# sparisi/pvr_habitat

Hardware: AMD Instinct MI355X
Metric: frames/sec embedded (ResNet50, 256x256) (higher is better)
Workload: dtype f16; 1 GPU; configs[1]: ResNet50 (MoCo-v2 layout) frozen, 256x256 uint8 frames resident in HBM, batch 256/GPU, random-init synthetic weights, f16 storage / MFMA inputs with fp32 accumulation (the product default, inside the 1e-3 parity bound; configs[1] names bf16); global_batch=256, frame=256, chunk=256, batches_in_flight=2, parallelism=frame shards, no collective (dp1)

## Files before the change

pvr_habitat_amd/csrc/bottleneck_chain.hip:

```cpp
#include "encoder_internal.h"

namespace pvr {


__device__ __forceinline__ void ch_dma16(__amdgpu_buffer_rsrc_t rs, char *lds, int voff, int soff) {
    __builtin_amdgcn_raw_ptr_buffer_load_lds(rs, (__attribute__((address_space(3))) void *)lds, 16, voff, soff, 0, 0);
}

#ifdef CHAIN_STAMP
__device__ unsigned long long chain_stamps[8192][12];
#define CH_T(i_) { if (threadIdx.x == 0) ch_tt[i_] = __builtin_amdgcn_s_memrealtime(); }
#else
#define CH_T(i_)
#endif

#ifndef CH_KNOCK
#define CH_KNOCK 0
#endif
template <int AUX = 0>
__device__ __forceinline__ void store_b128_imm(u32x4 v, __amdgpu_buffer_rsrc_t rs, int voff, int imm) {
    if constexpr (!(CH_KNOCK & 1)) __builtin_amdgcn_raw_buffer_store_b128(v, rs, voff + imm, 0, AUX);
}

template <int CM, int CMN, bool F16, int RD, int OCC, bool HALO, bool DS = false, int PFK = -1>
__global__ __launch_bounds__(256, OCC) void bottleneck_chain_kernel(ChainP p) {
    typedef typename HT<F16>::V8 V8;
    constexpr int BM = 128, BK = 64, BN = CM;
    constexpr int A_CH = BM / 32, B_CH = BN / 32, TM = 4, TN = BN / 32;
    constexpr int KS = CM / 64, HROWS = CM == 64 ? 256 : 192, RL = CM == 64 ? 3 : 2;
    constexpr int HSL = HROWS * 128, RING_OFF = KS * HSL, SLICE = CM * 128, ZERO_OFF = (HROWS - 1) * 128;
    constexpr int HOPS = KS * HROWS / 32;
    constexpr int STAGE = HALO ? (RING_OFF + 2 * SLICE) / 2 : (BM + BN) * 128;
    constexpr int C4 = 4 * CM, G = C4 / 64, KS3 = CM / 64;
    constexpr int TN1 = CMN / 32;
    constexpr int W3_CH = CM / 32, W1_CH = CMN / 32;
    constexpr int T2_OFF = 0;
    constexpr int YG_OFF = KS3 * 16384;
    constexpr int W3_OFF = YG_OFF + 16384;
    constexpr int W1_OFF = W3_OFF + KS3 * 8192;
    static_assert(W3_OFF + KS3 * 8192 <= 2 * STAGE, "phase-B tiles must fit the phase-A area");
    static_assert(RD >= 1 && RD <= G, "residual prefetch depth");
    extern __shared__ __attribute__((aligned(16))) char smem[];

    const int tid = threadIdx.x, lane = tid & 63, wave = tid >> 6;
#ifdef CHAIN_STAMP
    unsigned long long ch_tt[12] = {0, 0, 0, 0, 0, 0, 0, 0, 0, 0, 0, 0};
#endif
    CH_T(0);
    const int m0 = xcd_remap(blockIdx.x, gridDim.x) * BM;
    const int srow = tid >> 3, pch = tid & 7;
    const auto rs_in = __builtin_amdgcn_make_buffer_rsrc(const_cast<u16 *>(p.in), 0, p.in_bytes, 0x00020000);
    const auto rs_w2 = __builtin_amdgcn_make_buffer_rsrc(const_cast<u16 *>(p.w2), 0, p.w2_bytes, 0x00020000);
    const auto rs_w3 = __builtin_amdgcn_make_buffer_rsrc(const_cast<u16 *>(p.w3), 0, p.w3_bytes, 0x00020000);
    const auto rs_w1 = __builtin_amdgcn_make_buffer_rsrc(const_cast<u16 *>(p.w1n), 0, p.w1n_bytes, 0x00020000);
    const auto rs_res = __builtin_amdgcn_make_buffer_rsrc(const_cast<u16 *>(DS ? p.xds : p.res), 0, DS ? p.xds_bytes : p.y_bytes, 0x00020000);
    const auto rs_wd = __builtin_amdgcn_make_buffer_rsrc(const_cast<u16 *>(DS ? p.wds : p.w3), 0, DS ? p.wds_bytes : p.w3_bytes, 0x00020000);
    const auto rs_y = __builtin_amdgcn_make_buffer_rsrc(p.y, 0, p.y_bytes, 0x00020000);
    const auto rs_t = __builtin_amdgcn_make_buffer_rsrc(p.t1n, 0, p.t1n_bytes, 0x00020000);
    constexpr int OOB = 0x7ffffff0;

    if constexpr (HALO) {
        const int HR = 128 + 2 * p.W + 2, hbase = m0 - p.W - 1;
#pragma unroll
        for (int i = 0; i < HOPS; ++i) {
            const int o = i * 4 + wave, sl = o / (HROWS / 8), rb = o % (HROWS / 8);
            const int r = rb * 8 + (lane >> 3), c = (lane & 7) ^ (r & 6);
            const int vo = (r < HR && hbase + r >= 0) ? ((hbase + r) * CM + sl * 64 + c * 8) * 2 : OOB;
            ch_dma16(rs_in, smem + sl * HSL + rb * 1024, vo, 0);
        }
    }

    int a_off[A_CH], a_mask[A_CH];
#pragma unroll
    for (int i = 0; i < A_CH; ++i) {
        const int row = srow + 32 * i;
        const int lch = pch ^ ((row >> 1) & 7);
        const int m = m0 + row;
        const bool ok = m < p.M;
        const int mm = ok ? m : 0;
        const int wo = mm % p.Wo, t = mm / p.Wo, ho = t % p.Ho, n = t / p.Ho;
        const int hi0 = ho * p.stride - 1, wi0 = wo * p.stride - 1;
        a_off[i] = (((n * p.H + hi0) * p.W + wi0) * CM + lch * 8) * 2;
        int hb = 0, wb = 0;
#pragma unroll
        for (int t3 = 0; t3 < 3; ++t3) {
            hb |= (int)(ok && (unsigned)(hi0 + t3) < (unsigned)p.H) << t3;
            wb |= (int)((unsigned)(wi0 + t3) < (unsigned)p.W) << t3;
        }
        int mask = 0;
#pragma unroll
        for (int t3 = 0; t3 < 3; ++t3) mask |= ((hb >> t3) & 1) ? (wb << (t3 * 3)) : 0;
        a_mask[i] = mask;
    }
    int b_off[B_CH];
#pragma unroll
    for (int i = 0; i < B_CH; ++i) {
        const int row = srow + 32 * i;
        b_off[i] = (row * (9 * CM) + (pch ^ ((row >> 1) & 7)) * 8) * 2;
    }
    const int lds_st = srow * 128 + pch * 16;
    u32x4 ra[A_CH], rb[B_CH];
    constexpr int cpt = CM / BK, nk = 9 * cpt;
    int kh = 0, kw = 0, cs = 0, tap = 0;
#define PVR_LOAD_SLICE(kt_)                                                                             \
    {                                                                                                   \
        const int tap_off = ((kh * p.W + kw) * CM + cs * BK) * 2;                                       \
        _Pragma("unroll") for (int i = 0; i < A_CH; ++i) {                                              \
            const int vo = ((a_mask[i] >> tap) & 1) ? a_off[i] + tap_off : OOB;                         \
            ra[i] = __builtin_bit_cast(u32x4, __builtin_amdgcn_raw_buffer_load_b128(rs_in, vo, 0, 0));  \
        }                                                                                               \
        _Pragma("unroll") for (int i = 0; i < B_CH; ++i)                                                \
            rb[i] = __builtin_bit_cast(u32x4, __builtin_amdgcn_raw_buffer_load_b128(rs_w2, b_off[i], (kt_) * (BK * 2), 0)); \
        if (++cs == cpt) { cs = 0; ++tap; if (++kw == 3) { kw = 0; ++kh; } }                            \
    }
#define PVR_STORE_SLICE(buf_)                                                                           \
    {                                                                                                   \
        char *base = smem + (buf_) * STAGE + lds_st;                                                    \
        _Pragma("unroll") for (int i = 0; i < A_CH; ++i)                                                \
            *reinterpret_cast<u32x4 *>(base + i * 32 * 128) = ra[i];                                    \
        _Pragma("unroll") for (int i = 0; i < B_CH; ++i)                                                \
            *reinterpret_cast<u32x4 *>(base + BM * 128 + i * 32 * 128) = rb[i];                         \
    }

    const int wm = wave >> 1, wn = wave & 1;
    const int fr = lane & 15, fq = lane >> 4;
    int x_rd[2][TM];
    int b_rd[2][TN];
#pragma unroll
    for (int ks = 0; ks < 2; ++ks) {
#pragma unroll
        for (int j = 0; j < TM; ++j) {
            const int row = wm * 64 + j * 16 + fr;
            x_rd[ks][j] = row * 128 + (((ks * 4 + fq) ^ ((row >> 1) & 7)) << 4);
        }
#pragma unroll
        for (int i = 0; i < TN; ++i) {
            const int row = wn * (BN / 2) + i * 16 + fr;
            b_rd[ks][i] = BM * 128 + row * 128 + (((ks * 4 + fq) ^ ((row >> 1) & 7)) << 4);
        }
    }

    const int y_nhwc = ((m0 + wm * 64 + fr) * C4 + wn * 32 + fq * 8) * 2;
    const int y_blkd = ((m0 >> 4) + wm * 4) * (C4 * 32) + (wn * 4 + fq) * 256 + fr * 16;
    const int y_off0 = p.y_blk ? y_blkd : y_nhwc, y_js = p.y_blk ? C4 * 32 : 16 * C4 * 2, y_gs = p.y_blk ? 2048 : 128;
    const int r_off0 = p.res_blk ? y_blkd : y_nhwc, r_js = p.res_blk ? C4 * 32 : 16 * C4 * 2, r_gs = p.res_blk ? 2048 : 128;
    const int t_nhwc = ((m0 + wm * 64 + fr) * CMN + wn * (CMN / 2) + fq * 8) * 2;
    const int t_blkd = ((m0 >> 4) + wm * 4) * (CMN * 32) + (wn * (CMN / 16) + fq) * 256 + fr * 16;
    const int t_off0 = p.t_blk ? t_blkd : t_nhwc, t_js = p.t_blk ? CMN * 32 : 16 * CMN * 2;
#define Y_OFF(j_) (y_off0 + (j_) * y_js)
#define R_OFF(j_) (r_off0 + (j_) * r_js)
#define T_OFF(j_) (t_off0 + (j_) * t_js)
    const int st_r = tid >> 3, st_c = ((tid & 7) ^ ((st_r >> 1) & 7)) * 16;
    const int w3_g0 = st_r * CM * 2 + st_c, w3_l0 = W3_OFF + st_r * 128 + (tid & 7) * 16;
    const int w1_g0 = st_r * C4 * 2 + st_c, w1_l0 = W1_OFF + st_r * 128 + (tid & 7) * 16;
#define W3_G(i_) (w3_g0 + ((i_) & 1) * (32 * CM * 2) + ((i_) >> 1) * 128)
#define W3_L(i_) (w3_l0 + ((i_) & 1) * 4096 + ((i_) >> 1) * 8192)
#define W1_G(i_) (w1_g0 + (i_) * (32 * C4 * 2))
#define W1_L(i_) (w1_l0 + (i_) * 4096)
    u32x4 rres[RD][TM], w3r[W3_CH], w1r[CMN ? W1_CH : 1];
#define PVR_PHASE_B_PREFETCH()                                                                                          \
    {                                                                                                                   \
        if constexpr (!DS) {                                                                                            \
            _Pragma("unroll") for (int d = 0; d < RD; ++d)                                                              \
                _Pragma("unroll") for (int j = 0; j < TM; ++j)                                                          \
                    rres[d][j] = __builtin_bit_cast(u32x4, __builtin_amdgcn_raw_buffer_load_b128(rs_res, (CH_KNOCK & 2) ? OOB : R_OFF(j), d * r_gs, DS ? 0 : PVR_NT_AUX(16))); \
        }                                                                                                               \
        _Pragma("unroll") for (int i = 0; i < W3_CH; ++i)                                                               \
            w3r[i] = __builtin_bit_cast(u32x4, __builtin_amdgcn_raw_buffer_load_b128(rs_w3, W3_G(i), 0, 0));            \
        if constexpr (CMN > 0) {                                                                                        \
            _Pragma("unroll") for (int i = 0; i < W1_CH; ++i)                                                           \
                w1r[i] = __builtin_bit_cast(u32x4, __builtin_amdgcn_raw_buffer_load_b128(rs_w1, W1_G(i), 0, 0));        \
        }                                                                                                               \
    }
    if constexpr (!HALO || PFK < 0) PVR_PHASE_B_PREFETCH();

    f32x4 acc2[TN][TM];
#pragma unroll
    for (int i = 0; i < TN; ++i)
#pragma unroll
        for (int j = 0; j < TM; ++j) acc2[i][j] = f32x4{0.f, 0.f, 0.f, 0.f};
    if constexpr (HALO) {
        u32x4 w2r[RL][B_CH];
#pragma unroll
        for (int q = 0; q < RL; ++q)
#pragma unroll
            for (int i = 0; i < B_CH; ++i)
                w2r[q][i] = __builtin_bit_cast(u32x4, __builtin_amdgcn_raw_buffer_load_b128(rs_w2, b_off[i], q * (BK * 2), 0));
        asm volatile("s_waitcnt vmcnt(0)" ::: "memory");
#pragma unroll
        for (int i = 0; i < B_CH; ++i) *reinterpret_cast<u32x4 *>(smem + RING_OFF + lds_st + i * 32 * 128) = w2r[0][i];
        __syncthreads();
        CH_T(1);
        int h_row[TM], h_mask[TM];
#pragma unroll
        for (int j = 0; j < TM; ++j) {
            const int pr = wm * 64 + j * 16 + fr, m = m0 + pr;
            const bool ok = m < p.M;
            const int mm = ok ? m : 0;
            const int wo = mm % p.W, ho = (mm / p.W) % p.H;
            int hb = 0, wb_ = 0;
#pragma unroll
            for (int t3 = 0; t3 < 3; ++t3) {
                hb |= (int)(ok && (unsigned)(ho - 1 + t3) < (unsigned)p.H) << t3;
                wb_ |= (int)((unsigned)(wo - 1 + t3) < (unsigned)p.W) << t3;
            }
            int mask = 0;
#pragma unroll
            for (int t3 = 0; t3 < 3; ++t3) mask |= ((hb >> t3) & 1) ? (wb_ << (t3 * 3)) : 0;
            h_row[j] = pr; h_mask[j] = mask;
        }
#pragma unroll
        for (int kt = 0; kt < nk; ++kt) {
            if (kt == PFK) PVR_PHASE_B_PREFETCH();
            if (kt + RL < nk) {
#pragma unroll
                for (int i = 0; i < B_CH; ++i)
                    w2r[kt % RL][i] = __builtin_bit_cast(u32x4, __builtin_amdgcn_raw_buffer_load_b128(rs_w2, (CH_KNOCK & 8) ? OOB : b_off[i], (kt + RL) * (BK * 2), 0));
            }
            const int tp = kt / KS, csl = kt % KS, shift = (tp / 3) * p.W + tp % 3;
            int xo[TM];
#pragma unroll
            for (int j = 0; j < TM; ++j) {
                const int r = h_row[j] + shift;
                const int a = csl * HSL + r * 128 + ((fq ^ (r & 6)) << 4);
                xo[j] = ((h_mask[j] >> tp) & 1) ? a : ZERO_OFF;
            }
            const char *ring = smem + RING_OFF + (kt & 1) * SLICE - BM * 128;
#pragma unroll
            for (int ks = 0; ks < 2; ++ks) {
                V8 xa[TM], wb[TN];
#pragma unroll
                for (int j = 0; j < TM; ++j) if constexpr (!(CH_KNOCK & 32)) xa[j] = *reinterpret_cast<const V8 *>(smem + (xo[j] ^ (ks * 64)));
#pragma unroll
                for (int i = 0; i < TN; ++i) if constexpr (!(CH_KNOCK & 32)) wb[i] = *reinterpret_cast<const V8 *>(ring + b_rd[ks][i]);
#pragma unroll
                for (int i = 0; i < TN; ++i)
#pragma unroll
                    for (int j = 0; j < TM; ++j) acc2[i][j] = mfma16<F16>(wb[i], xa[j], acc2[i][j]);
            }
            if (kt + 1 < nk) {
#pragma unroll
                for (int i = 0; i < B_CH; ++i)
                    if constexpr (!(CH_KNOCK & 4)) *reinterpret_cast<u32x4 *>(smem + RING_OFF + ((kt + 1) & 1) * SLICE + lds_st + i * 32 * 128) = w2r[(kt + 1) % RL][i];
            }
            if constexpr (!(CH_KNOCK & 16)) __syncthreads();
        }
    } else {
    PVR_LOAD_SLICE(0);
    PVR_STORE_SLICE(0);
    __syncthreads();
    CH_T(1);
#define PVR_K_STEP(kt_, CUR_)                                                                           \
    {                                                                                                   \
        const bool more = (kt_) + 1 < nk;                                                               \
        if (more) PVR_LOAD_SLICE((kt_) + 1);                                                            \
        const char *sb = smem + (CUR_) * STAGE;                                                         \
        _Pragma("unroll") for (int ks = 0; ks < 2; ++ks) {                                              \
            V8 xa[TM], wb[TN];                                                                          \
            _Pragma("unroll") for (int j = 0; j < TM; ++j) xa[j] = *reinterpret_cast<const V8 *>(sb + x_rd[ks][j]); \
            _Pragma("unroll") for (int i = 0; i < TN; ++i) wb[i] = *reinterpret_cast<const V8 *>(sb + b_rd[ks][i]); \
            _Pragma("unroll") for (int i = 0; i < TN; ++i)                                              \
                _Pragma("unroll") for (int j = 0; j < TM; ++j) acc2[i][j] = mfma16<F16>(wb[i], xa[j], acc2[i][j]); \
        }                                                                                               \
        if (more) PVR_STORE_SLICE(1 - (CUR_));                                                          \
        __syncthreads();                                                                                \
    }
    for (int kt = 0; kt < nk; kt += 2) {
        PVR_K_STEP(kt, 0);
        if (kt + 1 < nk) PVR_K_STEP(kt + 1, 1);
    }
    }
    CH_T(2);
    V8 xd[2][TM], wdr[2][2];
    int wd_off[2];
    if constexpr (DS) {
#pragma unroll
        for (int j = 0; j < TM; ++j) {
            const int xo_ = (m0 + wm * 64 + j * 16 + fr) * 128 + fq * 16;
#pragma unroll
            for (int ks = 0; ks < 2; ++ks) xd[ks][j] = __builtin_bit_cast(V8, __builtin_amdgcn_raw_buffer_load_b128(rs_res, xo_, ks * 64, 0));
        }
#pragma unroll
        for (int t = 0; t < 2; ++t) {
            wd_off[t] = (wn * 32 + t * 16 + fr) * 128 + fq * 16;
#pragma unroll
            for (int ks = 0; ks < 2; ++ks) wdr[t][ks] = __builtin_bit_cast(V8, __builtin_amdgcn_raw_buffer_load_b128(rs_wd, wd_off[t] + ks * 64, 0, 0));
        }
    }
#undef PVR_K_STEP
#undef PVR_LOAD_SLICE
#undef PVR_STORE_SLICE

#pragma unroll
    for (int i = 0; i < TN; ++i) {
        const int c = wn * (BN / 2) + i * 16 + fq * 4;
        const float4 bv = *reinterpret_cast<const float4 *>(p.b2 + c);
#pragma unroll
        for (int j = 0; j < TM; ++j) {
            const int row = wm * 64 + j * 16 + fr;
            const f32x4 a = acc2[i][j];
            const unsigned lo = pack2_h<F16>(fmaxf(a[0] + bv.x, 0.f), fmaxf(a[1] + bv.y, 0.f));
            const unsigned hi = pack2_h<F16>(fmaxf(a[2] + bv.z, 0.f), fmaxf(a[3] + bv.w, 0.f));
            const int cc = c & 63;
            char *dst = smem + T2_OFF + (c >> 6) * 16384 + row * 128 + ((((cc >> 3) ^ ((row >> 1) & 7))) << 4) + (cc & 4) * 2;
            *reinterpret_cast<uint2 *>(dst) = make_uint2(lo, hi);
        }
    }
#pragma unroll
    for (int i = 0; i < W3_CH; ++i) *reinterpret_cast<u32x4 *>(smem + W3_L(i)) = w3r[i];
    if constexpr (CMN > 0) {
#pragma unroll
        for (int i = 0; i < W1_CH; ++i) *reinterpret_cast<u32x4 *>(smem + W1_L(i)) = w1r[i];
    }
    if (G > 1) {
#pragma unroll
        for (int i = 0; i < W3_CH; ++i)
            w3r[i] = __builtin_bit_cast(u32x4, __builtin_amdgcn_raw_buffer_load_b128(rs_w3, W3_G(i), 64 * CM * 2, 0));
        if constexpr (CMN > 0) {
#pragma unroll
            for (int i = 0; i < W1_CH; ++i) w1r[i] = __builtin_bit_cast(u32x4, __builtin_amdgcn_raw_buffer_load_b128(rs_w1, W1_G(i), 128, 0));
        }
    }
    __syncthreads();
    CH_T(3);

    int w3_rd[2][2], w1_rd[2][CMN ? TN1 : 1], yg_wr[TM];
#pragma unroll
    for (int ks = 0; ks < 2; ++ks) {
#pragma unroll
        for (int t = 0; t < 2; ++t) {
            const int row = wn * 32 + t * 16 + fr;
            w3_rd[ks][t] = W3_OFF + row * 128 + (((ks * 4 + fq) ^ ((row >> 1) & 7)) << 4);
        }
        if constexpr (CMN > 0) {
#pragma unroll
            for (int i = 0; i < TN1; ++i) {
                const int row = wn * (CMN / 2) + i * 16 + fr;
                w1_rd[ks][i] = W1_OFF + row * 128 + (((ks * 4 + fq) ^ ((row >> 1) & 7)) << 4);
            }
        }
    }
#pragma unroll
    for (int j = 0; j < TM; ++j) {
        const int row = wm * 64 + j * 16 + fr;
        yg_wr[j] = YG_OFF + row * 128 + (((wn * 4 + fq) ^ ((row >> 1) & 7)) << 4);
    }
    f32x4 acc1[CMN ? TN1 : 1][TM];
    if constexpr (CMN > 0) {
#pragma unroll
        for (int i = 0; i < TN1; ++i)
#pragma unroll
            for (int j = 0; j < TM; ++j) acc1[i][j] = f32x4{0.f, 0.f, 0.f, 0.f};
    }

#pragma unroll
    for (int g = 0; g < G; ++g) {
        if (g == 1) CH_T(6);
        f32x4 acc3[2][TM];
#pragma unroll
        for (int t = 0; t < 2; ++t)
#pragma unroll
            for (int j = 0; j < TM; ++j) acc3[t][j] = f32x4{0.f, 0.f, 0.f, 0.f};
#pragma unroll
        for (int s = 0; s < KS3; ++s)
#pragma unroll
            for (int ks = 0; ks < 2; ++ks) {
                V8 xa[TM], wb[2];
#pragma unroll
                for (int j = 0; j < TM; ++j) xa[j] = *reinterpret_cast<const V8 *>(smem + T2_OFF + s * 16384 + x_rd[ks][j]);
#pragma unroll
                for (int t = 0; t < 2; ++t) wb[t] = *reinterpret_cast<const V8 *>(smem + s * 8192 + w3_rd[ks][t]);
#pragma unroll
                for (int t = 0; t < 2; ++t)
#pragma unroll
                    for (int j = 0; j < TM; ++j) acc3[t][j] = mfma16<F16>(wb[t], xa[j], acc3[t][j]);
            }
        if constexpr (DS) {
#pragma unroll
            for (int ks = 0; ks < 2; ++ks)
#pragma unroll
                for (int t = 0; t < 2; ++t)
#pragma unroll
                    for (int j = 0; j < TM; ++j) acc3[t][j] = mfma16<F16>(wdr[t][ks], xd[ks][j], acc3[t][j]);
            if (g + 1 < G) {
#pragma unroll
                for (int t = 0; t < 2; ++t)
#pragma unroll
                    for (int ks = 0; ks < 2; ++ks)
                        wdr[t][ks] = __builtin_bit_cast(V8, __builtin_amdgcn_raw_buffer_load_b128(rs_wd, wd_off[t] + ks * 64, (g + 1) * 8192, 0));
            }
        }
        if (g == 1) CH_T(7);
        const int c0 = g * 64 + wn * 32 + fq * 8;
        const float4 bA = *reinterpret_cast<const float4 *>(p.b3 + c0), bB = *reinterpret_cast<const float4 *>(p.b3 + c0 + 4);
#pragma unroll
        for (int j = 0; j < TM; ++j) {
            const f32x4 lo = acc3[0][j], hi = acc3[1][j];
            float v[8] = {lo[0] + bA.x, lo[1] + bA.y, lo[2] + bA.z, lo[3] + bA.w, hi[0] + bB.x, hi[1] + bB.y, hi[2] + bB.z, hi[3] + bB.w};
            u32x4 o;
            if constexpr (DS) {
#pragma unroll
                for (int e = 0; e < 4; ++e)
                    o[e] = pack2_h<F16>(fmaxf(v[2 * e], 0.f), fmaxf(v[2 * e + 1], 0.f));
            } else {
                const u32x4 r = rres[g % RD][j];
#pragma unroll
                for (int e = 0; e < 4; ++e) {
                    const float v0 = fmaxf(v[2 * e] + from_h<F16>((u16)(r[e] & 0xffffu)), 0.f);
                    const float v1 = fmaxf(v[2 * e + 1] + from_h<F16>((u16)(r[e] >> 16)), 0.f);
                    o[e] = pack2_h<F16>(v0, v1);
                }
            }
            if (p.y_blk) store_b128_imm<PVR_NT_AUX(4)>(o, rs_y, Y_OFF(j) + g * y_gs, 0);
            else store_b128_imm(o, rs_y, Y_OFF(j) + g * y_gs, 0);
            if constexpr (CMN > 0) *reinterpret_cast<u32x4 *>(smem + yg_wr[j]) = o;
        }
        if (!DS && g + RD < G) {
#pragma unroll
            for (int j = 0; j < TM; ++j)
                rres[g % RD][j] = __builtin_bit_cast(u32x4, __builtin_amdgcn_raw_buffer_load_b128(rs_res, (CH_KNOCK & 2) ? OOB : R_OFF(j), (g + RD) * r_gs, DS ? 0 : PVR_NT_AUX(16)));
        }
        if (g == 1) CH_T(8);
        __syncthreads();
        if (g == 1) CH_T(9);
        if (g + 1 < G) {
#pragma unroll
            for (int i = 0; i < W3_CH; ++i) *reinterpret_cast<u32x4 *>(smem + W3_L(i)) = w3r[i];
            if (g + 2 < G) {
#pragma unroll
                for (int i = 0; i < W3_CH; ++i)
                    w3r[i] = __builtin_bit_cast(u32x4, __builtin_amdgcn_raw_buffer_load_b128(rs_w3, W3_G(i), (g + 2) * (64 * CM * 2), 0));
            }
        }
        if (g == 1) CH_T(10);
        if constexpr (CMN == 0) __syncthreads();
        if constexpr (CMN > 0) {
#pragma unroll
            for (int ks = 0; ks < 2; ++ks) {
                V8 xa[TM], wb[TN1];
#pragma unroll
                for (int j = 0; j < TM; ++j) xa[j] = *reinterpret_cast<const V8 *>(smem + YG_OFF + x_rd[ks][j]);
#pragma unroll
                for (int i = 0; i < TN1; ++i) wb[i] = *reinterpret_cast<const V8 *>(smem + w1_rd[ks][i]);
#pragma unroll
                for (int i = 0; i < TN1; ++i)
#pragma unroll
                    for (int j = 0; j < TM; ++j) acc1[i][j] = mfma16<F16>(wb[i], xa[j], acc1[i][j]);
            }
            __syncthreads();
            if (g == 1) CH_T(11);
            if (g + 1 < G) {
#pragma unroll
                for (int i = 0; i < W1_CH; ++i) *reinterpret_cast<u32x4 *>(smem + W1_L(i)) = w1r[i];
                if (g + 2 < G) {
#pragma unroll
                    for (int i = 0; i < W1_CH; ++i)
                        w1r[i] = __builtin_bit_cast(u32x4, __builtin_amdgcn_raw_buffer_load_b128(rs_w1, W1_G(i), (g + 2) * 128, 0));
                }
            }
        }
    }

    CH_T(4);
    if constexpr (CMN > 0) {
#pragma unroll
        for (int q = 0; q < TN1 / 2; ++q) {
            const int c0 = wn * (CMN / 2) + q * 32 + fq * 8;
            const float4 bA = *reinterpret_cast<const float4 *>(p.b1n + c0), bB = *reinterpret_cast<const float4 *>(p.b1n + c0 + 4);
#pragma unroll
            for (int j = 0; j < TM; ++j) {
                const f32x4 lo = acc1[2 * q][j], hi = acc1[2 * q + 1][j];
                const float v[8] = {lo[0] + bA.x, lo[1] + bA.y, lo[2] + bA.z, lo[3] + bA.w, hi[0] + bB.x, hi[1] + bB.y, hi[2] + bB.z, hi[3] + bB.w};
                u32x4 o;
#pragma unroll
                for (int e = 0; e < 4; ++e)
                    o[e] = pack2_h<F16>(fmaxf(v[2 * e], 0.f), fmaxf(v[2 * e + 1], 0.f));
                if (p.t_blk) store_b128_imm<0>(o, rs_t, T_OFF(j) + q * 1024, 0);
                else store_b128_imm<PVR_NT_AUX(8)>(o, rs_t, T_OFF(j), q * 64);
            }
        }
    }
#undef PVR_PHASE_B_PREFETCH
#undef W3_G
#undef W3_L
#undef W1_G
#undef W1_L
#undef Y_OFF
#undef R_OFF
#undef T_OFF
#ifdef CHAIN_STAMP
    CH_T(5);
    if (threadIdx.x == 0 && blockIdx.x < 8192) { _Pragma("unroll") for (int k = 0; k < 12; ++k) chain_stamps[blockIdx.x][k] = ch_tt[k]; }
#endif
}

template <int CM, int CMN, bool F16, int RD, int OCC, bool HALO, bool DS = false, int PFK = -1>
static pvr_status launch_chain_one(ChainP &p, hipStream_t stream) {
    const int grid = (p.M + 127) / 128;
    const size_t pipe = HALO ? (size_t)(CM / 64) * (CM == 64 ? 256 : 192) * 128 + (size_t)2 * CM * 128 : (size_t)2 * (128 + CM) * 128;
    const size_t phase_b = (CM / 64) * 16384 + 16384 + (CM / 64) * 8192 + CMN * 128;
    const size_t lds = phase_b <= pipe ? pipe : phase_b;
    static DeviceOnce attr_done;
    if (attr_done.needed()) {
        PVR_HIP_TRY(hipFuncSetAttribute((const void *)bottleneck_chain_kernel<CM, CMN, F16, RD, OCC, HALO, DS, PFK>,
                                        hipFuncAttributeMaxDynamicSharedMemorySize, (int)lds));
        attr_done.mark();
    }
    hipLaunchKernelGGL((bottleneck_chain_kernel<CM, CMN, F16, RD, OCC, HALO, DS, PFK>), dim3(grid), dim3(256), lds, stream, p);
    PVR_LAUNCH_CHECK();
    return PVR_OK;
}

template <int CM, int CMN, bool F16, int RD, int OCC, bool DS = false>
static pvr_status launch_chain_inst(ChainP &p, const PlanSwitches &sw, hipStream_t stream) {
    const bool halo = p.stride == 1 && 128 + 2 * p.W + 2 <= (CM == 64 ? 256 : 192) - 1 && sw.chain_halo;
    if constexpr (DS) {
        if (halo) return sw.chain_ds_occ == 3 ? launch_chain_one<CM, CMN, F16, RD, 3, true, true>(p, stream) : launch_chain_one<CM, CMN, F16, RD, 2, true, true>(p, stream);
        return launch_chain_one<CM, CMN, F16, RD, 2, false, true>(p, stream);
    } else {
        if (halo) {
            if constexpr (CM == 128) {
                if (sw.chain_pfk == 12) return launch_chain_one<CM, CMN, F16, RD, 2, true, false, 12>(p, stream);
            }
            return launch_chain_one<CM, CMN, F16, RD, (CM == 64 ? OCC : 2), true>(p, stream);
        }
        return launch_chain_one<CM, CMN, F16, RD, OCC, false>(p, stream);
    }
}

template <bool F16>
static pvr_status launch_chain_dt(ChainP &p, int cm, int cmn, const PlanSwitches &sw, hipStream_t stream) {
    if (p.xds) {
        if (cm == 64 && cmn == 64) return launch_chain_inst<64, 64, F16, 1, 2, true>(p, sw, stream);
        set_error("bottleneck chain with downsample: no instance for Cm=%d, next Cm=%d", cm, cmn);
        return PVR_ERR_INVALID;
    }
    const int cfg = sw.chain_cfg;
#define PVR_CHAIN64(CMN_)                                                                 \
    switch (cfg) {                                                                        \
    case 12: return launch_chain_inst<64, CMN_, F16, 1, 2>(p, sw, stream);                \
    case 13: return launch_chain_inst<64, CMN_, F16, 1, 3>(p, sw, stream);                \
    case 22: return launch_chain_inst<64, CMN_, F16, 2, 2>(p, sw, stream);                \
    case 23: return launch_chain_inst<64, CMN_, F16, 2, 3>(p, sw, stream);                \
    default: return launch_chain_inst<64, CMN_, F16, 4, 2>(p, sw, stream);                \
    }
    if (cm == 64 && cmn == 64) PVR_CHAIN64(64)
    if (cm == 64 && cmn == 128) {
        if (cfg / 10 == 1) return launch_chain_inst<64, 128, F16, 1, 2>(p, sw, stream);
        if (cfg / 10 == 2) return launch_chain_inst<64, 128, F16, 2, 2>(p, sw, stream);
        return launch_chain_inst<64, 128, F16, 4, 2>(p, sw, stream);
    }
    if (cm == 64 && cmn == 0) PVR_CHAIN64(0)
#undef PVR_CHAIN64
    if (cm == 128 && cmn == 128) return launch_chain_inst<128, 128, F16, 1, 2>(p, sw, stream);
    if (cm == 128 && cmn == 0) return launch_chain_inst<128, 0, F16, 1, 2>(p, sw, stream);
    set_error("bottleneck chain: no instance for Cm=%d, next Cm=%d", cm, cmn);
    return PVR_ERR_INVALID;
}

bool chain_uses_wave_form(const PlanSwitches &sw, int cm, int cmn, int stride, bool ds) { return sw.chain_wave && chain_wave_supported(sw, cm, cmn, stride, ds); }

bool chain_ds_supported(int cm, int cmn, int cin, int stride) { return cm == 64 && cmn == 64 && cin == 64 && stride == 1; }
bool chain_supported(int cm, int cmn) { return (cm == 64 && (cmn == 0 || cmn == 64 || cmn == 128)) || (cm == 128 && (cmn == 0 || cmn == 128)); }

int chain_row_source(int row) { return (row & ~31) + 8 * ((row >> 2) & 3) + 4 * ((row >> 4) & 1) + (row & 3); }

pvr_status launch_bottleneck_chain(const PlanSwitches &sw, const void *t1, const void *w2, const float *b2, const void *w3p, const float *b3, const void *res,
                                   void *y, const void *w1np, const float *b1n, void *t1n, int n, int h, int w, int cm, int cmn,
                                   int stride, int dtype, hipStream_t stream, const void *xds, const void *wdsp, const void *w3pb, const void *wdspb,
                                   int wave, int in_blk, int out_blk, int y_s2) {
    PVR_REQUIRE(chain_supported(cm, cmn), "bottleneck chain: unsupported widths Cm=%d next=%d", cm, cmn);
    PVR_REQUIRE(t1 && w2 && b2 && w3p && b3 && (res || xds) && y && (cmn == 0 || (w1np && b1n && t1n)), "bottleneck chain: null argument");
    PVR_REQUIRE(!xds || (wdsp && chain_ds_supported(cm, cmn, 64, stride)), "bottleneck chain with downsample: unsupported shape");
    ChainP p;
    p.in = (const u16 *)t1; p.w2 = (const u16 *)w2; p.w3 = (const u16 *)w3p; p.w1n = (const u16 *)w1np; p.res = (const u16 *)res;
    p.b2 = b2; p.b3 = b3; p.b1n = b1n; p.y = (u16 *)y; p.t1n = (u16 *)t1n;
    p.N = n; p.H = h; p.W = w; p.stride = stride;
    p.Ho = (h + 2 - 3) / stride + 1; p.Wo = (w + 2 - 3) / stride + 1;
    const int64_t M = (int64_t)n * p.Ho * p.Wo;
    const int64_t inb = (int64_t)n * h * w * cm * 2, yb = M * 4 * cm * 2, tb = M * (cmn ? cmn : 1) * 2;
    PVR_REQUIRE(inb < 0x7ffffff0ll && yb < 0x7ffffff0ll && tb < 0x7ffffff0ll, "bottleneck chain: operand larger than 2 GiB (use a smaller chunk)");
    p.M = (int)M; p.in_bytes = (unsigned)inb; p.y_bytes = (unsigned)yb; p.t1n_bytes = (unsigned)tb;
    p.xds = (const u16 *)xds; p.wds = (const u16 *)wdsp;
    p.xds_bytes = xds ? (unsigned)(M * 64 * 2) : 0; p.wds_bytes = xds ? (unsigned)(4 * cm * 64 * 2) : 0;
    p.w2_bytes = (unsigned)(cm * 9 * cm * 2); p.w3_bytes = (unsigned)(4 * cm * cm * 2); p.w1n_bytes = (unsigned)(cmn * 4 * cm * 2);
    if (wave) {
        PVR_REQUIRE(chain_wave_supported(sw, cm, cmn, stride, xds != nullptr), "bottleneck chain: no wave form for Cm=%d next=%d stride=%d", cm, cmn, stride);
        p.w3b = (const u16 *)w3pb; p.wdsb = (const u16 *)wdspb; p.in_blk = in_blk; p.out_blk = out_blk; p.y_s2 = y_s2;
        return launch_chain_wave(p, cmn, sw.chain_wave_halo, dtype, stream);
    }
    PVR_REQUIRE(!y_s2, "bottleneck chain: y_s2 is a store of the wave form");
    PVR_REQUIRE(!(in_blk || out_blk) || M % 16 == 0, "bottleneck chain: the blocked layout needs a multiple of 16 pixels");
    p.res_blk = xds ? 0 : in_blk; p.y_blk = out_blk;
    return dtype == PVR_F16 ? launch_chain_dt<true>(p, cm, cmn, sw, stream) : launch_chain_dt<false>(p, cm, cmn, sw, stream);
}

}
```

pvr_habitat_amd/csrc/encoder.hip:

```cpp
#include "encoder_internal.h"

namespace pvr {

pvr_status launch_split16_pack(const float *w, void *out, int rows, int K, hipStream_t stream);
pvr_status launch_conv_split16(const float *in, const void *wsp, const float *bias, const float *res, float *out, int n, int h, int w, int cin,
                               int cout, int k, int stride, int pad, int relu, hipStream_t stream, float *out2 = nullptr, int n1 = 0, void *out16 = nullptr,
                               int terms = 3);

void read_switches(PlanSwitches &sw) {
    auto get = [](const char *name, int def) { const char *v = getenv(name); return v ? atoi(v) : def; };
    sw.pool_fuse = get("PVR_POOL_FUSE", 1);
    sw.stem_u8 = get("PVR_STEM_U8", 1);
    sw.stem_lds = get("PVR_STEM_LDS", 1);
    sw.stem_regpool = get("PVR_STEM_REGPOOL", 1);
    sw.frame_front1 = get("PVR_FRAME_FRONT1", 1);
    sw.frame_next1 = get("PVR_FRAME_NEXT1", 0);
    sw.frame_bneck = get("PVR_FRAME_BNECK", 1);
    sw.bneck_stagger = get("PVR_FRAME_STAGGER", 0);
    sw.dual_ds = get("PVR_DUAL_DS", 1);
    sw.chain_ds = get("PVR_CHAIN_DS", 1);
    sw.chain_blocked = get("PVR_CHAIN_BLOCKED", 1);
    sw.chain_halo = get("PVR_CHAIN_HALO", 1);
    sw.chain_ds_occ = get("PVR_CHAIN_DS_OCC", 3);
    sw.chain_pfk = get("PVR_CHAIN_PFK", 12);
    sw.chain_cfg = get("PVR_CHAIN_CFG", 12);
    sw.chain_wave = get("PVR_CHAIN_WAVE", 1);
    sw.chain_wave_halo = get("PVR_CHAIN_WAVE_HALO", 1);
    sw.chain_wave_128 = get("PVR_CHAIN_WAVE_128", 1);
    sw.strided_y = get("PVR_STRIDED_Y", 1);
    sw.splitk = get("PVR_SPLITK", 1);
    sw.smallk_div = get("PVR_SMALLK_DIV", 4);
    if (sw.smallk_div < 1) sw.smallk_div = 1;
    sw.frame_min_n = get("PVR_FRAME_MIN_N", 128);
    sw.frame_run = get("PVR_FRAME_RUN", 0);
    sw.frame_stagger = get("PVR_FRAME_RUN_STAGGER", 0);
    sw.split16 = get("PVR_SPLIT16", 1);
    sw.stem_conv1 = get("PVR_STEM_CONV1", 1);
    sw.resid32 = get("PVR_RESID32", 1);
    sw.tail_f32 = get("PVR_TAIL_F32", 1);
    sw.fuse = get("PVR_FUSE", 1);
    sw.conv_algo = get("PVR_CONV_ALGO", -1);
    sw.conv_halo = get("PVR_CONV_HALO", 1);
    sw.conv_expand = get("PVR_CONV_EXPAND", 1);
    sw.conv_wfrag = get("PVR_CONV_WFRAG", 1);
    sw.wfrag_ko = get("PVR_WFRAG_KO", 0);
    sw.igemm_nk4 = get("PVR_IGEMM_NK4", 1);
    sw.igemm_bm64 = get("PVR_IGEMM_BM64", 0);
    sw.pp_bm224 = get("PVR_PP_BM224", 1);
    sw.pp_persist = get("PVR_PP_PERSIST", 384);
}

PlanSwitches &op_switches() {
    static PlanSwitches sw = [] { PlanSwitches v; read_switches(v); return v; }();
    return sw;
}

template <bool F32>
__global__ __launch_bounds__(256) void range_flag_kernel(const void *x, size_t n8, int dtype, int *flags, int idx) {
    bool bad = false;
    for (size_t i = (size_t)blockIdx.x * 256 + threadIdx.x; i < n8; i += (size_t)gridDim.x * 256) {
        if constexpr (F32) {
            const u32x4 a = reinterpret_cast<const u32x4 *>(x)[2 * i], b = reinterpret_cast<const u32x4 *>(x)[2 * i + 1];
#pragma unroll
            for (int e = 0; e < 4; ++e) bad |= (a[e] & 0x7f800000u) == 0x7f800000u || (b[e] & 0x7f800000u) == 0x7f800000u;
        } else {
            const u32x4 a = reinterpret_cast<const u32x4 *>(x)[i];
            const unsigned em = dtype == PVR_F16 ? 0x7c00u : 0x7f80u;
#pragma unroll
            for (int e = 0; e < 4; ++e) bad |= ((a[e] & em) == em) || (((a[e] >> 16) & em) == em);
        }
    }
    if (__builtin_amdgcn_ballot_w64(bad) != 0 && (threadIdx.x & 63) == 0) atomicOr(flags + idx, 1);
}

__global__ __launch_bounds__(256) void range_flag_split_kernel(const float *x, size_t n4, int *flags, int idx) {
    bool bad = false;
    for (size_t i = (size_t)blockIdx.x * 256 + threadIdx.x; i < n4; i += (size_t)gridDim.x * 256) {
        const u32x4 a = reinterpret_cast<const u32x4 *>(x)[i];
#pragma unroll
        for (int e = 0; e < 4; ++e) bad |= (a[e] & 0x7fffffffu) > 0x477fe000u;
    }
    if (__builtin_amdgcn_ballot_w64(bad) != 0 && (threadIdx.x & 63) == 0) atomicOr(flags + idx, 1);
}
static void launch_range_flag_split(const void *x, size_t elems, int *flags, int idx, hipStream_t st) {
    const size_t n4 = elems / 4;
    hipLaunchKernelGGL(range_flag_split_kernel, dim3((unsigned)((n4 + 255) / 256 < 2048 ? (n4 + 255) / 256 : 2048)), dim3(256), 0, st, (const float *)x, n4, flags, idx);
}

const HostTensor *enc_find(pvr_encoder *e, const std::string &name) {
    auto it = e->weights.find(name);
    return it == e->weights.end() ? nullptr : &it->second;
}

pvr_status enc_need(pvr_encoder *e, const std::string &name, const HostTensor **out, size_t numel) {
    const HostTensor *t = enc_find(e, name);
    if (!t) { set_error("missing weight: %s", name.c_str()); return PVR_ERR_MISSING_WEIGHT; }
    if (t->data.size() != numel) {
        set_error("weight %s has %zu elements, expected %zu", name.c_str(), t->data.size(), numel);
        return PVR_ERR_INVALID;
    }
    *out = t;
    return PVR_OK;
}

static pvr_status bn_fold(pvr_encoder *e, const std::string &bn, int c, std::vector<float> &scale,
                          std::vector<float> &shift) {
    const HostTensor *g, *b, *m, *v;
    pvr_status s;
    if ((s = enc_need(e, bn + ".weight", &g, c))) return s;
    if ((s = enc_need(e, bn + ".bias", &b, c))) return s;
    if ((s = enc_need(e, bn + ".running_mean", &m, c))) return s;
    if ((s = enc_need(e, bn + ".running_var", &v, c))) return s;
    scale.resize(c); shift.resize(c);
    for (int i = 0; i < c; ++i) {
        scale[i] = g->data[i] / sqrtf(v->data[i] + 1e-5f);
        shift[i] = b->data[i] - m->data[i] * scale[i];
    }
    return PVR_OK;
}


static pvr_status finalize_conv(pvr_encoder *e, ConvOp &op) {
    const int k = op.k, cr = op.cin_real, cor = op.cout_real;
    const HostTensor *w;
    pvr_status s;
    if ((s = enc_need(e, op.conv + ".weight", &w, (size_t)cor * cr * k * k))) return s;
    std::vector<float> scale, shift;
    if ((s = bn_fold(e, op.bn, cor, scale, shift))) return s;
    if (const HostTensor *cb = enc_find(e, op.conv + ".bias")) {
        if ((int)cb->data.size() != cor) { set_error("bad bias size for %s", op.conv.c_str()); return PVR_ERR_INVALID; }
        for (int i = 0; i < cor; ++i) shift[i] += scale[i] * cb->data[i];
    }
    const int cout_pad = (op.cout + 63) / 64 * 64;
    const size_t K = (size_t)k * k * op.cin;
    std::vector<u16> hw(cout_pad * K, 0);
    for (int co = 0; co < cor; ++co)
        for (int ci = 0; ci < cr; ++ci)
            for (int a = 0; a < k; ++a)
                for (int b = 0; b < k; ++b) {
                    const float v = w->data[(((size_t)co * cr + ci) * k + a) * k + b] * scale[co];
                    hw[co * K + ((size_t)a * k + b) * op.cin + ci] = f32_to_h(v, e->desc.dtype);
                }
    std::vector<float> hb(cout_pad, 0.f);
    for (int co = 0; co < cor; ++co) hb[co] = shift[co];
    if (stores_f32(e->desc.dtype) || op.f32op || op.from32) {
        std::vector<float> hf(cout_pad * K, 0.f);
        for (int co = 0; co < cor; ++co)
            for (int ci = 0; ci < cr; ++ci)
                for (int a = 0; a < k; ++a)
                    for (int b = 0; b < k; ++b)
                        hf[co * K + ((size_t)a * k + b) * op.cin + ci] = w->data[(((size_t)co * cr + ci) * k + a) * k + b] * scale[co];
        if ((s = enc_upload(&op.d_wf, hf))) return s;
        if (op.split16) {
            PVR_HIP_TRY(hipMalloc((void **)&op.d_wsp, (size_t)cout_pad * K * 4));
            if ((s = launch_split16_pack(op.d_wf, op.d_wsp, cout_pad, (int)K, nullptr))) return s;
        }
        if (op.from32 && !op.split16) { set_error("%s: a convolution that reads the fp32 stream needs the conv_split16 weight image (cin %d, cout %d)", op.conv.c_str(), op.cin, op.cout); return PVR_ERR_INVALID; }
        op.h_b = hb;
        return enc_upload(&op.d_b, hb);
    }
    if ((s = enc_upload(&op.d_w, hw))) return s;
    op.h_w = std::move(hw);
    op.h_b = hb;
    return enc_upload(&op.d_b, hb);
}

static pvr_status pack_wfb(ConvOp &o) {
    if (o.d_wfb) return PVR_OK;
    const size_t K = (size_t)o.k * o.k * o.cin;
    PVR_HIP_TRY(hipMalloc((void **)&o.d_wfb, (size_t)o.cout * K * 2));
    return launch_pack_frag_weights(o.d_w, o.d_wfb, o.cout, (int)K, nullptr);
}

static pvr_status prepare_weights(pvr_encoder *e) {
    pvr_status s;
    for (ConvOp &op : e->ops)
        if (op.wfrag && (s = pack_wfb(op))) return s;
// ... 866 lines not shown
```

pvr_habitat_amd/csrc/encoder_internal.h:

```cpp
#pragma once
#include <map>
#include <string>
#include <vector>
#include <cmath>
#include "common.h"
#include "chain_params.h"

namespace pvr {

struct PlanSwitches {
    int pool_fuse = 1;
    int stem_u8 = 1;
    int stem_lds = 1;
    int stem_regpool = 1;
    int frame_front1 = 1;
    int frame_next1 = 0;
    int frame_bneck = 1;
    int bneck_stagger = 0;
    int dual_ds = 1;
    int chain_ds = 1;
    int chain_blocked = 1;
    int chain_halo = 1;
    int chain_ds_occ = 3;
    int chain_pfk = 12;
    int chain_cfg = 12;
    int chain_wave = 1;
    int chain_wave_halo = 1;
    int chain_wave_128 = 1;
    int strided_y = 1;
    int splitk = 1;
    int smallk_div = 4;
    int frame_run = 0;
    int frame_stagger = 0;
    int frame_min_n = 128;
    int stem_conv1 = 1;
    int split16 = 1;
    int resid32 = 1;
    int tail_f32 = 1;
    int fuse = 1;
    int conv_algo = -1;
    int conv_halo = 1;
    int conv_expand = 1;
    int conv_wfrag = 1;
    int wfrag_ko = 0;
    int igemm_nk4 = 1;
    int igemm_bm64 = 0;
    int pp_bm224 = 1;
    int pp_persist = 384;
};
void read_switches(PlanSwitches &sw);
PlanSwitches &op_switches();

pvr_status launch_preprocess(const uint8_t *, int, int, int, int, int, void *, int, hipStream_t, int crop_pos = 0);
pvr_status launch_stem(const void *, const void *, const float *, void *, int, int, int, hipStream_t);
pvr_status launch_maxpool(const void *, void *, int, int, int, int, int, hipStream_t);
pvr_status launch_stem_pool(const PlanSwitches &sw, const void *, const void *, const float *, void *, int, int, int, hipStream_t, const void *c1_w = nullptr,
                            const float *c1_b = nullptr, void *c1_t1 = nullptr, int c1_blk = 0);
bool stem_pool_u8_ok(const void *, int, int, int, int);
pvr_status launch_stem_pool_u8(const PlanSwitches &sw, const uint8_t *, int, int, int, int, int, const void *, const float *, void *, int, hipStream_t,
                               const void *c1_w = nullptr, const float *c1_b = nullptr, void *c1_t1 = nullptr, int c1_blk = 0);
bool stem_conv1_capable(const PlanSwitches &sw);
void stem_c1_pack(const u16 *w, u16 *img);
void preprocess_geometry(int h, int w, int resize, int crop, int crop_pos, int *resize_needed, int *top, int *left);
pvr_status launch_avgpool(const void *, float *, int64_t, int, int, int, int, int, hipStream_t);
pvr_status launch_nhwc_to_chw(const float *, float *, int64_t, int, int, int, int, hipStream_t);
pvr_status launch_h_to_f32(const void *, float *, size_t, int, hipStream_t);
pvr_status launch_f32_to_h(const float *, void *, size_t, int, hipStream_t);
pvr_status launch_conv_splitk(const void *, const void *, const float *, const void *, void *, const void *, float *, int, int, int, int, int, int,
                              int, int, int, int, int, int, int, hipStream_t);
pvr_status launch_conv(const PlanSwitches &sw, const void *, const void *, const float *, const void *, void *, const void *, int, int, int, int,
                       int, int, int, int, int, int, int, int, hipStream_t);

bool conv_expand_supported(const PlanSwitches &sw, int64_t M, int h, int w, int cin, int cout, int kh, int kw, int stride, int pad, int relu, int out_f32, bool has_res);
pvr_status launch_conv_expand(const void *in, const void *wgt, const float *bias, const void *res, void *out, int n, int h, int w, int cin,
                              int cout, int stride, int relu, int dtype, hipStream_t stream, int out_blk = 0);

bool pp256_supported(int64_t M, int cin, int cout, int kh, int kw, int64_t in_bytes, int64_t w_bytes, int64_t out_bytes, int64_t res_bytes);
pvr_status launch_conv_pp256(const PlanSwitches &sw, const void *in, const void *wgt, const float *bias, const void *res, void *out, int n, int h, int w, int cin,
                             int cout, int kh, int kw, int stride, int pad, int act, int out_f32, int res_f32, int dtype, int bm, hipStream_t stream,
                             const void *in2 = nullptr, int h2 = 0, int w2 = 0, int cin2 = 0, int stride2 = 1);

bool bneck_frame_supported(const PlanSwitches &sw, int n, int h, int w, int cm, int cout, int stride);
pvr_status launch_pack_frag_weights(const void *w, void *out, int rows, int K, hipStream_t stream);
pvr_status launch_bneck_frame(const PlanSwitches &sw, const void *t1, const void *w2p, const float *b2, const void *w3p, const float *b3, const void *res, void *y,
                              void *t2_out, int n, int phases, int dtype, hipStream_t stream, unsigned long long *stamps = nullptr,
                              const void *w1np = nullptr, const float *b1n = nullptr, void *t1n = nullptr, const void *w1fp = nullptr, const float *b1f = nullptr);
struct BFBlk {
    const unsigned short *w1f, *w2, *w3, *res;
    const float *b1f, *b2, *b3;
    unsigned short *y;
};
pvr_status launch_bneck_frame_run(const BFBlk *blocks, int nblk, int n, int dtype, hipStream_t stream, int stagger);

bool conv_wfrag_supported(int64_t M, int64_t in_bytes, int cin, int cout, int kh, int kw, int pad, int act, int out_f32);
bool conv_wfrag_preferred(const PlanSwitches &sw, int64_t M, int cin, int cout, int kh, int kw);
pvr_status launch_conv_wfrag(const PlanSwitches &sw, const void *in, const void *wp, const float *bias, const void *res, void *out, int n, int h, int w, int cin, int cout,
                             int kh, int kw, int stride, int pad, int act, int out_f32, int dtype, hipStream_t stream, float *pool_out = nullptr,
                             int64_t pool_stride = 0);

struct HostTensor {
    std::vector<int64_t> shape;
    std::vector<float> data;
};

inline bool stores_f32(int dtype) { return dtype == PVR_F32 || dtype == PVR_F32S; }

constexpr int PVR_MAX_LANES = 4;
enum BufId { B_NONE = -1, B_X0 = 0, B_X1, B_T1, B_T2, B_DS, B_F32, B_Y0, B_Y1, B_COUNT, B_STEM = B_COUNT };

enum OpRole : uint8_t {
    R_CONV1, R_CONV2, R_CONV3, R_DOWNSAMPLE,
    R_HEAD_CONV1, R_HEAD_DOWNSAMPLE, R_HEAD_CONV2,
    R_STEM_CONV2, R_STEM_CONV3,
    R_AVGPOOL2,
    R_CAST,
};

inline int conv_out_size(int in, int k, int stride, int pad) { return (in + 2 * pad - k) / stride + 1; }

struct ConvOp {
    std::string conv, bn;
    OpRole role = R_CONV1;
    int in_buf, out_buf, res_buf;
    int h, w, cin, cin_real, cout, cout_real, k, stride, pad, relu, out_f32;
    bool is_conv() const { return role < R_AVGPOOL2; }
    int ho() const { return conv_out_size(h, k, stride, pad); }
    int wo() const { return conv_out_size(w, k, stride, pad); }
    bool f32op = false;
    bool from32 = false;
    bool split16 = false;
    bool wfrag = false;
    u16 *d_w = nullptr;
    u16 *d_wp = nullptr;
    u16 *d_wfb = nullptr;
    u16 *d_wpb = nullptr;
    std::vector<u16> h_w;
    float *d_wf = nullptr;
    u16 *d_wsp_pair = nullptr;
    float *d_b_pair = nullptr;
    u16 *d_wsp = nullptr;
    float *d_b = nullptr;
    std::vector<float> h_b;
    float *d_bsum = nullptr;
    u16 *d_wcat = nullptr;
    std::string tap;
    int ksplit = 0, ks_buf = B_NONE;
};

enum BlockType : uint8_t { BK_BOTTLENECK, BK_BASIC, BK_HEAD };
struct Block {
    BlockType type;
    int stage, index;
    int conv1 = -1, conv2 = -1, ds = -1, conv3 = -1;
    int cast = -1;
};

enum LaunchForm : uint8_t {
    LF_SINGLE,
    LF_CHAIN,
    LF_FRAME,
    LF_DUAL,
    LF_PAIR,
};
struct Launch {
    LaunchForm form = LF_SINGLE;
    int conv2 = -1, conv3 = -1, next1 = -1;
    int ds = -1;
    int t1_in = B_NONE, t1_out = B_NONE;
    int wave = 0;
    int conv1 = -1;
    int pair = -1;
    int in_blk = 0, out_blk = 0;
    int y_s2 = -1;
    int out_op() const { return form == LF_CHAIN || form == LF_FRAME ? conv3 : conv2; }
};

enum LaunchKind : uint8_t {
// ... 135 lines not shown
```

Baseline: 98120 frames/s.

## Spread residual prefetch across phase-A k-steps and specialize Cm=128 chain epilogue

Adds an optional schedule for the Cm=128 bottleneck chain that issues residual loads one at a time, spaced across phase-A k-steps, instead of in a single batch before the loop. The depth is chosen by a new PVR_CHAIN_RD switch. The change also makes the y-store cache policy a compile-time choice and software-prefetches the next group's bias during the epilogue. When PFK is set, the phase-A loop is fully unrolled so the prefetch point can sit at any k-step. The aim is to hide residual and bias load latency behind MFMA work, at the cost of more kernel instances and higher register pressure from deeper prefetch.

```diff
diff --git a/pvr_habitat_amd/csrc/bottleneck_chain.hip b/pvr_habitat_amd/csrc/bottleneck_chain.hip
--- a/pvr_habitat_amd/csrc/bottleneck_chain.hip
+++ b/pvr_habitat_amd/csrc/bottleneck_chain.hip
@@ -22,7 +22,7 @@
     if constexpr (!(CH_KNOCK & 1)) __builtin_amdgcn_raw_buffer_store_b128(v, rs, voff + imm, 0, AUX);
 }
 
-template <int CM, int CMN, bool F16, int RD, int OCC, bool HALO, bool DS = false, int PFK = -1>
+template <int CM, int CMN, bool F16, int RD, int OCC, bool HALO, bool DS = false, int PFK = -1, int RS = -1, int YB = -1>
 __global__ __launch_bounds__(256, OCC) void bottleneck_chain_kernel(ChainP p) {
     typedef typename HT<F16>::V8 V8;
     constexpr int BM = 128, BK = 64, BN = CM;
@@ -40,6 +40,8 @@
     constexpr int W1_OFF = W3_OFF + KS3 * 8192;
     static_assert(W3_OFF + KS3 * 8192 <= 2 * STAGE, "phase-B tiles must fit the phase-A area");
     static_assert(RD >= 1 && RD <= G, "residual prefetch depth");
+    constexpr int NKA = 9 * (CM / BK), RSTEP = RS < 0 ? 1 : ((NKA - 2 - RS) / (RD * TM) > 1 ? (NKA - 2 - RS) / (RD * TM) : 1);
+    static_assert(RS < 0 || (!DS && PFK >= 0 && RS + (RD * TM - 1) * RSTEP < NKA), "every ring request is issued inside phase A");
     extern __shared__ __attribute__((aligned(16))) char smem[];
 
     const int tid = threadIdx.x, lane = tid & 63, wave = tid >> 6;
@@ -160,7 +162,7 @@
     u32x4 rres[RD][TM], w3r[W3_CH], w1r[CMN ? W1_CH : 1];
 #define PVR_PHASE_B_PREFETCH()                                                                                          \
     {                                                                                                                   \
-        if constexpr (!DS) {                                                                                            \
+        if constexpr (!DS && RS < 0) {                                                                                  \
             _Pragma("unroll") for (int d = 0; d < RD; ++d)                                                              \
                 _Pragma("unroll") for (int j = 0; j < TM; ++j)                                                          \
                     rres[d][j] = __builtin_bit_cast(u32x4, __builtin_amdgcn_raw_buffer_load_b128(rs_res, (CH_KNOCK & 2) ? OOB : R_OFF(j), d * r_gs, DS ? 0 : PVR_NT_AUX(16))); \
@@ -172,7 +174,13 @@
                 w1r[i] = __builtin_bit_cast(u32x4, __builtin_amdgcn_raw_buffer_load_b128(rs_w1, W1_G(i), 0, 0));        \
         }                                                                                                               \
     }
-    if constexpr (!HALO || PFK < 0) PVR_PHASE_B_PREFETCH();
+    if constexpr (PFK < 0) PVR_PHASE_B_PREFETCH();
+#define PVR_RING_REQUEST(kt_)                                                                                           \
+    if constexpr (RS >= 0) {                                                                                            \
+        const int q_ = ((kt_) - RS) / RSTEP;                                                                            \
+        if ((kt_) >= RS && ((kt_) - RS) % RSTEP == 0 && q_ < RD * TM)                                                   \
+            rres[q_ / TM][q_ % TM] = __builtin_bit_cast(u32x4, __builtin_amdgcn_raw_buffer_load_b128(rs_res, (CH_KNOCK & 2) ? OOB : R_OFF(q_ % TM), (q_ / TM) * r_gs, PVR_NT_AUX(16))); \
+    }
 
     f32x4 acc2[TN][TM];
 #pragma unroll
@@ -237,6 +245,7 @@
                 for (int i = 0; i < TN; ++i)
 #pragma unroll
                     for (int j = 0; j < TM; ++j) acc2[i][j] = mfma16<F16>(wb[i], xa[j], acc2[i][j]);
+                if (ks == 0) PVR_RING_REQUEST(kt);
             }
             if (kt + 1 < nk) {
 #pragma unroll
@@ -261,13 +270,22 @@
             _Pragma("unroll") for (int i = 0; i < TN; ++i) wb[i] = *reinterpret_cast<const V8 *>(sb + b_rd[ks][i]); \
             _Pragma("unroll") for (int i = 0; i < TN; ++i)                                              \
                 _Pragma("unroll") for (int j = 0; j < TM; ++j) acc2[i][j] = mfma16<F16>(wb[i], xa[j], acc2[i][j]); \
+            if (ks == 0) PVR_RING_REQUEST(kt_);                                                         \
         }                                                                                               \
         if (more) PVR_STORE_SLICE(1 - (CUR_));                                                          \
         __syncthreads();                                                                                \
     }
+    if constexpr (PFK >= 0) {
+#pragma unroll
+        for (int kt = 0; kt < nk; ++kt) {
+            if (kt == PFK) PVR_PHASE_B_PREFETCH();
+            PVR_K_STEP(kt, kt & 1);
+        }
+    } else {
     for (int kt = 0; kt < nk; kt += 2) {
         PVR_K_STEP(kt, 0);
         if (kt + 1 < nk) PVR_K_STEP(kt + 1, 1);
+    }
     }
     }
     CH_T(2);
@@ -353,9 +371,17 @@
             for (int j = 0; j < TM; ++j) acc1[i][j] = f32x4{0.f, 0.f, 0.f, 0.f};
     }
 
+    constexpr bool BPF = YB >= 0;
+    const int b3_c0 = wn * 32 + fq * 8;
+    float4 bAn = make_float4(0.f, 0.f, 0.f, 0.f), bBn = bAn;
+    if constexpr (BPF) { bAn = *reinterpret_cast<const float4 *>(p.b3 + b3_c0); bBn = *reinterpret_cast<const float4 *>(p.b3 + b3_c0 + 4); }
 #pragma unroll
     for (int g = 0; g < G; ++g) {
         if (g == 1) CH_T(6);
+        const float4 bAc = bAn, bBc = bBn;
+        if constexpr (BPF) {
+            if (g + 1 < G) { bAn = *reinterpret_cast<const float4 *>(p.b3 + (g + 1) * 64 + b3_c0); bBn = *reinterpret_cast<const float4 *>(p.b3 + (g + 1) * 64 + b3_c0 + 4); }
+        }
         f32x4 acc3[2][TM];
 #pragma unroll
         for (int t = 0; t < 2; ++t)
@@ -392,7 +418,7 @@
         }
         if (g == 1) CH_T(7);
         const int c0 = g * 64 + wn * 32 + fq * 8;
-        const float4 bA = *reinterpret_cast<const float4 *>(p.b3 + c0), bB = *reinterpret_cast<const float4 *>(p.b3 + c0 + 4);
+        const float4 bA = BPF ? bAc : *reinterpret_cast<const float4 *>(p.b3 + c0), bB = BPF ? bBc : *reinterpret_cast<const float4 *>(p.b3 + c0 + 4);
 #pragma unroll
         for (int j = 0; j < TM; ++j) {
             const f32x4 lo = acc3[0][j], hi = acc3[1][j];
@@ -411,7 +437,9 @@
                     o[e] = pack2_h<F16>(v0, v1);
                 }
             }
-            if (p.y_blk) store_b128_imm<PVR_NT_AUX(4)>(o, rs_y, Y_OFF(j) + g * y_gs, 0);
+            if constexpr (YB == 1) store_b128_imm<PVR_NT_AUX(4)>(o, rs_y, Y_OFF(j) + g * y_gs, 0);
+            else if constexpr (YB == 0) store_b128_imm(o, rs_y, Y_OFF(j) + g * y_gs, 0);
+            else if (p.y_blk) store_b128_imm<PVR_NT_AUX(4)>(o, rs_y, Y_OFF(j) + g * y_gs, 0);
             else store_b128_imm(o, rs_y, Y_OFF(j) + g * y_gs, 0);
             if constexpr (CMN > 0) *reinterpret_cast<u32x4 *>(smem + yg_wr[j]) = o;
         }
@@ -481,6 +509,7 @@
         }
     }
 #undef PVR_PHASE_B_PREFETCH
+#undef PVR_RING_REQUEST
 #undef W3_G
 #undef W3_L
 #undef W1_G
@@ -494,7 +523,7 @@
 #endif
 }
 
-template <int CM, int CMN, bool F16, int RD, int OCC, bool HALO, bool DS = false, int PFK = -1>
+template <int CM, int CMN, bool F16, int RD, int OCC, bool HALO, bool DS = false, int PFK = -1, int RS = -1, int YB = -1>
 static pvr_status launch_chain_one(ChainP &p, hipStream_t stream) {
     const int grid = (p.M + 127) / 128;
     const size_t pipe = HALO ? (size_t)(CM / 64) * (CM == 64 ? 256 : 192) * 128 + (size_t)2 * CM * 128 : (size_t)2 * (128 + CM) * 128;
@@ -502,29 +531,35 @@
     const size_t lds = phase_b <= pipe ? pipe : phase_b;
     static DeviceOnce attr_done;
     if (attr_done.needed()) {
-        PVR_HIP_TRY(hipFuncSetAttribute((const void *)bottleneck_chain_kernel<CM, CMN, F16, RD, OCC, HALO, DS, PFK>,
+        PVR_HIP_TRY(hipFuncSetAttribute((const void *)bottleneck_chain_kernel<CM, CMN, F16, RD, OCC, HALO, DS, PFK, RS, YB>,
                                         hipFuncAttributeMaxDynamicSharedMemorySize, (int)lds));
         attr_done.mark();
     }
-    hipLaunchKernelGGL((bottleneck_chain_kernel<CM, CMN, F16, RD, OCC, HALO, DS, PFK>), dim3(grid), dim3(256), lds, stream, p);
+    hipLaunchKernelGGL((bottleneck_chain_kernel<CM, CMN, F16, RD, OCC, HALO, DS, PFK, RS, YB>), dim3(grid), dim3(256), lds, stream, p);
     PVR_LAUNCH_CHECK();
     return PVR_OK;
 }
 
-template <int CM, int CMN, bool F16, int RD, int OCC, bool DS = false>
+template <int CM, int CMN, bool F16, int RD, int OCC, bool DS = false, bool CW = false>
 static pvr_status launch_chain_inst(ChainP &p, const PlanSwitches &sw, hipStream_t stream) {
     const bool halo = p.stride == 1 && 128 + 2 * p.W + 2 <= (CM == 64 ? 256 : 192) - 1 && sw.chain_halo;
     if constexpr (DS) {
         if (halo) return sw.chain_ds_occ == 3 ? launch_chain_one<CM, CMN, F16, RD, 3, true, true>(p, stream) : launch_chain_one<CM, CMN, F16, RD, 2, true, true>(p, stream);
         return launch_chain_one<CM, CMN, F16, RD, 2, false, true>(p, stream);
     } else {
-        if (halo) {
-            if constexpr (CM == 128) {
-                if (sw.chain_pfk == 12) return launch_chain_one<CM, CMN, F16, RD, 2, true, false, 12>(p, stream);
-            }
-            return launch_chain_one<CM, CMN, F16, RD, (CM == 64 ? OCC : 2), true>(p, stream);
-        }
-        return launch_chain_one<CM, CMN, F16, RD, OCC, false>(p, stream);
+        if constexpr (CM == 128 && CW) {
+            constexpr int RS = RD == 1 ? -1 : RD == 4 ? 0 : 1, PFH = RD == 1 ? 12 : 16, PFT = RD == 1 ? -1 : 16;
+            if (halo) return p.y_blk ? launch_chain_one<CM, CMN, F16, RD, 2, true, false, PFH, RS, 1>(p, stream) : launch_chain_one<CM, CMN, F16, RD, 2, true, false, PFH, RS, 0>(p, stream);
+            return p.y_blk ? launch_chain_one<CM, CMN, F16, RD, 2, false, false, PFT, RS, 1>(p, stream) : launch_chain_one<CM, CMN, F16, RD, 2, false, false, PFT, RS, 0>(p, stream);
+        } else {
+            if (halo) {
+                if constexpr (CM == 128) {
+                    if (sw.chain_pfk == 12) return launch_chain_one<CM, CMN, F16, RD, 2, true, false, 12>(p, stream);
+                }
+                return launch_chain_one<CM, CMN, F16, RD, (CM == 64 ? OCC : 2), true>(p, stream);
+            }
+            return launch_chain_one<CM, CMN, F16, RD, OCC, false>(p, stream);
+        }
     }
 }
 
@@ -552,8 +587,20 @@
     }
     if (cm == 64 && cmn == 0) PVR_CHAIN64(0)
 #undef PVR_CHAIN64
-    if (cm == 128 && cmn == 128) return launch_chain_inst<128, 128, F16, 1, 2>(p, sw, stream);
-    if (cm == 128 && cmn == 0) return launch_chain_inst<128, 0, F16, 1, 2>(p, sw, stream);
+    if (cm == 128 && (cmn == 128 || cmn == 0)) {
+        const int rd = cmn == 0 ? sw.chain_rd % 10 : p.stride == 1 ? sw.chain_rd / 10 % 10 : sw.chain_rd / 100 % 10;
+        if (cmn == 128) {
+            if (rd == 1) return launch_chain_inst<128, 128, F16, 1, 2, false, true>(p, sw, stream);
+            if (rd == 2) return launch_chain_inst<128, 128, F16, 2, 2, false, true>(p, sw, stream);
+            if (rd == 3) return launch_chain_inst<128, 128, F16, 3, 2, false, true>(p, sw, stream);
+            return launch_chain_inst<128, 128, F16, 1, 2>(p, sw, stream);
+        }
+        if (rd == 1) return launch_chain_inst<128, 0, F16, 1, 2, false, true>(p, sw, stream);
+        if (rd == 2) return launch_chain_inst<128, 0, F16, 2, 2, false, true>(p, sw, stream);
+        if (rd == 3) return launch_chain_inst<128, 0, F16, 3, 2, false, true>(p, sw, stream);
+        if (rd == 4) return launch_chain_inst<128, 0, F16, 4, 2, false, true>(p, sw, stream);
+        return launch_chain_inst<128, 0, F16, 1, 2>(p, sw, stream);
+    }
     set_error("bottleneck chain: no instance for Cm=%d, next Cm=%d", cm, cmn);
     return PVR_ERR_INVALID;
 }
diff --git a/pvr_habitat_amd/csrc/encoder.hip b/pvr_habitat_amd/csrc/encoder.hip
--- a/pvr_habitat_amd/csrc/encoder.hip
+++ b/pvr_habitat_amd/csrc/encoder.hip
@@ -23,6 +23,7 @@
     sw.chain_halo = get("PVR_CHAIN_HALO", 1);
     sw.chain_ds_occ = get("PVR_CHAIN_DS_OCC", 3);
     sw.chain_pfk = get("PVR_CHAIN_PFK", 12);
+    sw.chain_rd = get("PVR_CHAIN_RD", 1);
     sw.chain_cfg = get("PVR_CHAIN_CFG", 12);
     sw.chain_wave = get("PVR_CHAIN_WAVE", 1);
     sw.chain_wave_halo = get("PVR_CHAIN_WAVE_HALO", 1);
diff --git a/pvr_habitat_amd/csrc/encoder_internal.h b/pvr_habitat_amd/csrc/encoder_internal.h
--- a/pvr_habitat_amd/csrc/encoder_internal.h
+++ b/pvr_habitat_amd/csrc/encoder_internal.h
@@ -23,6 +23,7 @@
     int chain_halo = 1;
     int chain_ds_occ = 3;
     int chain_pfk = 12;
+    int chain_rd = 1;
     int chain_cfg = 12;
     int chain_wave = 1;
     int chain_wave_halo = 1;
```

Result: no change. 98220 frames/s, median of 6 (+0.1%).
